# krm01/Snappy.jl

Measured on AMD Instinct MI355X. Metric: GB/s compressed+decompressed (batched blocks) at 1/2/4/8 GPUs; % HBM peak, higher is better.
Workload: dtype u8; 1 GPU; configs 2+3: 10000 x 64 KiB text blocks per GPU, fast-mode compress + uncompress round trip per step; blocks_per_gpu=10000, block_bytes=65536, parallelism=dp1 (blocks sharded per rank, RCCL size all-gather)

## Files before the change

snappy.jl_amd/csrc/sm_compress_sc.hip:

```cpp
#include "sm_device.h"
#include "sm_internal.h"

namespace sm {

constexpr uint32_t kScS = 1024;
constexpr uint32_t kScC = kScS / 64;
constexpr uint32_t kScG = kScS / 64;
constexpr uint32_t kScW = 16;
constexpr uint32_t kScWorkers = kScW - 1;
#ifndef SC_RING
#define SC_RING 16
#endif
constexpr uint32_t kScRing = SC_RING;
static_assert((kScRing & (kScRing - 1)) == 0, "the span kernel's slot sequence needs a power of 2");
constexpr uint32_t kScSlot = 1088;
constexpr uint32_t kScThreads = 64 * kScW;
constexpr uint32_t kScTabBits = 13;
constexpr uint32_t kScTabWords = 1u << kScTabBits;
constexpr uint32_t kScExt = 17;
constexpr uint32_t kScMaxL = 255;
#ifndef SC_SPIN_BITS
#define SC_SPIN_BITS 22
#endif
constexpr uint32_t kScSpinMax = 1u << SC_SPIN_BITS;
static_assert(kScC == 16 && kScG == 16, "a lane's 16 positions: one u16 mask, one 16-byte row");

#ifndef SC_CB
#define SC_CB 2
#endif
#ifndef SC_FAR
#define SC_FAR 256
#endif
constexpr uint32_t kMaskPasses = 16;
#ifndef SC_WPRIO
#define SC_WPRIO 3
#endif
#ifndef SC_TPRIO
#define SC_TPRIO 3
#endif
#ifndef SC_TSLEEP
#define SC_TSLEEP 1
#endif
#ifndef SC_WSLEEP
#define SC_WSLEEP 1
#endif


struct ScWaveLds {
  uint8_t L[kScS];
  uint16_t O[kScS];
};
struct ScLds {
  uint8_t pre[16];
  uint8_t blk[kBlockSize + 64];
  uint32_t T[kScTabWords + 4];
  ScWaveLds w[kScWorkers];
  uint8_t ring[kScRing][kScSlot];
  uint32_t rsize[kScRing];
  uint32_t rseq[kScRing];
  uint32_t ins;
  uint32_t next;
  uint32_t err;
};
static_assert(sizeof(ScLds) <= 160 * 1024, "LDS");
static_assert(sizeof(ScWaveLds) % 32 == 0 && offsetof(ScLds, w) % 32 == 0 && offsetof(ScWaveLds, O) % 32 == 0,
              "rows are 32-byte aligned (section C's O addresses XOR the swizzle into bits 2..4)");
static_assert(kScSlot % 16 == 0 && offsetof(ScLds, ring) % 16 == 0, "slots are 16-byte aligned");
static_assert(kScSlot == kSpanSlot, "the host sizes part pitches by the staging slot");

template <typename Pred>
__device__ __attribute__((always_inline)) inline uint32_t sc_wait(uint32_t* p, Pred pred, uint32_t& err, uint32_t code) {
  uint32_t v;
  for (uint32_t it = 0; !pred(v = uniform(__hip_atomic_load(p, __ATOMIC_ACQUIRE, __HIP_MEMORY_SCOPE_WORKGROUP))); ++it) {
    if (it > kScSpinMax) {
      err |= code;
      break;
    }
    if (SC_WSLEEP) __builtin_amdgcn_s_sleep(SC_WSLEEP);
  }
  return v;
}


__device__ inline uint32_t sc_ld32(const uint8_t* blk, uint32_t a) { return *reinterpret_cast<const uint32_t*>(blk + a); }


__device__ inline uint32_t sc_abyte(uint32_t hi, uint32_t lo, uint32_t s) { return __builtin_amdgcn_alignbyte(hi, lo, s); }

__device__ inline uint32_t sc_ld32u(const uint8_t* blk, uint32_t p) {
  const uint32_t* w = reinterpret_cast<const uint32_t*>(blk + (p & ~3u));
  return sc_abyte(w[1], w[0], p);
}

__device__ inline uint4 sc_ld128(const uint8_t* blk, uint32_t p) {
  const uint32_t* w = reinterpret_cast<const uint32_t*>(blk + (p & ~3u));
  const uint32_t s = p;
  const uint32_t w0 = w[0], w1 = w[1], w2 = w[2], w3 = w[3], w4 = w[4];
  return make_uint4(__builtin_amdgcn_alignbyte(w1, w0, s), __builtin_amdgcn_alignbyte(w2, w1, s),
                    __builtin_amdgcn_alignbyte(w3, w2, s), __builtin_amdgcn_alignbyte(w4, w3, s));
}

__device__ inline uint32_t sc_diff8(uint32_t a0, uint32_t a1, uint32_t b0, uint32_t b1) {
  const uint64_t d = ((uint64_t)(a1 ^ b1) << 32) | (a0 ^ b0);
  return d ? (uint32_t)__builtin_ctzll(d) >> 3 : 8u;
}

__device__ inline uint4 sc_trim(uint4 v, uint32_t len) {
  const uint64_t mlo = len >= 8 ? ~0ull : (1ull << (8 * (len & 7))) - 1;
  const uint64_t mhi = len >= 16 ? ~0ull : (len <= 8 ? 0ull : (1ull << (8 * (len & 7))) - 1);
  return make_uint4(v.x & (uint32_t)mlo, v.y & (uint32_t)(mlo >> 32), v.z & (uint32_t)mhi, v.w & (uint32_t)(mhi >> 32));
}

__device__ inline uint4 sc_trim1(uint4 v, uint32_t len) {
  uint32_t l8 = len << 3;
  asm("" : "+v"(l8));
  uint64_t mlo, mhi;
  asm("v_lshrrev_b64 %0, %1, -1" : "=v"(mlo) : "v"(64 - min(l8, 64u)));
  asm("v_lshrrev_b64 %0, %1, -1" : "=v"(mhi) : "v"(128 - l8));
  const bool hi = len > 8;
  return make_uint4(v.x & (uint32_t)mlo, v.y & (uint32_t)(mlo >> 32), hi ? v.z & (uint32_t)mhi : 0u,
                    hi ? v.w & (uint32_t)(mhi >> 32) : 0u);
}

__device__ inline void sc_lds_or(uint32_t a, uint4 v) {
  const uint32_t wa = (a - 1u) & ~3u, t = 0u - a;
  const uint32_t u0 = __builtin_amdgcn_alignbyte(v.x, 0u, t);
  const uint32_t u1 = __builtin_amdgcn_alignbyte(v.y, v.x, t);
  const uint32_t u2 = __builtin_amdgcn_alignbyte(v.z, v.y, t);
  const uint32_t u3 = __builtin_amdgcn_alignbyte(v.w, v.z, t);
  const uint32_t u4 = __builtin_amdgcn_alignbyte(0u, v.w, t);
  asm volatile("ds_or_b32 %0, %1\nds_or_b32 %0, %2 offset:4\nds_or_b32 %0, %3 offset:8\nds_or_b32 %0, %4 offset:12\n"
               "ds_or_b32 %0, %5 offset:16"
               : : "v"(wa), "v"(u0), "v"(u1), "v"(u2), "v"(u3), "v"(u4) : "memory");
}

__device__ inline void sc_lds_orn(uint32_t a, uint4 v, uint32_t nb) {
  const uint32_t wa = (a - 1u) & ~3u, t = 0u - a, d = a - wa;
  const uint32_t u0 = __builtin_amdgcn_alignbyte(v.x, 0u, t);
  const uint32_t u1 = __builtin_amdgcn_alignbyte(v.y, v.x, t);
  asm volatile("ds_or_b32 %0, %1" : : "v"(wa), "v"(u0) : "memory");
  asm volatile("ds_or_b32 %0, %1 offset:4" : : "v"(wa), "v"(u1) : "memory");
  if (d + nb > 8) {
    const uint32_t u2 = __builtin_amdgcn_alignbyte(v.z, v.y, t);
    const uint32_t u3 = __builtin_amdgcn_alignbyte(v.w, v.z, t);
    const uint32_t u4 = __builtin_amdgcn_alignbyte(0u, v.w, t);
    asm volatile("ds_or_b32 %0, %1 offset:8\nds_or_b32 %0, %2 offset:12\nds_or_b32 %0, %3 offset:16"
                 : : "v"(wa), "v"(u2), "v"(u3), "v"(u4) : "memory");
  }
}

__device__ inline void sc_lds_or3(uint32_t a, uint32_t cv) {
  const uint32_t wa = (a - 1u) & ~3u, t = 0u - a;
  const uint32_t lo = __builtin_amdgcn_alignbyte(cv, 0u, t), hi = __builtin_amdgcn_alignbyte(0u, cv, t);
  asm volatile("ds_or_b32 %0, %1\nds_or_b32 %0, %2 offset:4" : : "v"(wa), "v"(lo), "v"(hi) : "memory");
}

__device__ inline uint4 sc_prepend(uint4 v, uint32_t tag, uint32_t t) {
  if (t == 0) return v;
  const uint32_t s = 4 - t;
  return make_uint4(__builtin_amdgcn_alignbyte(v.x, tag << (8 * s), s), __builtin_amdgcn_alignbyte(v.y, v.x, s),
                    __builtin_amdgcn_alignbyte(v.z, v.y, s), __builtin_amdgcn_alignbyte(v.w, v.z, s));
}

__device__ inline TagBytes sc_run_tag(uint32_t len) {
  __builtin_assume(len >= 1 && len <= kScS);
  return literal_tag(len, kLiteralStd);
}

__device__ inline uint32_t sc_hash_bucket(uint32_t w) {
  uint32_t h;
  asm("v_bfe_u32 %0, %1, %2, %3" : "=v"(h) : "v"(w * kHashMul), "n"(32 - kScTabBits), "n"(kScTabBits));
  return h;
}

__device__ inline uint32_t sc_select(uint64_t m, uint32_t a, uint32_t b) {
  uint32_t r;
  asm("v_cndmask_b32_e64 %0, %1, %2, %3" : "=v"(r) : "v"(b), "v"(a), "s"(m));
  return r;
}

__device__ inline uint32_t sc_sel(uint32_t c, uint32_t a, uint32_t b) { return c ? a : b; }

__device__ inline uint32_t sc_extend(const uint8_t* blk, uint32_t q, uint32_t off, uint32_t L, uint32_t cap) {
  for (;;) {
    const uint4 x = sc_ld128(blk, q + L), y = sc_ld128(blk, q + L - off);
    const uint32_t f0 = sc_diff8(x.x, x.y, y.x, y.y);
    const uint32_t fb = f0 < 8 ? f0 : 8u + sc_diff8(x.z, x.w, y.z, y.w);
    L = min(L + fb, cap);
    if (fb < 16 || L >= cap) return L;
  }
}

__device__ inline uint32_t sc_ffbl(uint32_t x) {
  uint32_t r;
  asm("v_ffbl_b32 %0, %1" : "=v"(r) : "v"(x));
  return r;
}

__device__ __attribute__((always_inline)) inline uint32_t sc_eq16(uint32_t X0, uint32_t X1, uint32_t X2, uint32_t X3,
                                                                  const uint32_t* w, uint32_t s) {
  const uint32_t a0 = w[0], a1 = w[1], a2 = w[2], a3 = w[3], a4 = w[4];
  const uint32_t b0 = sc_ffbl(X0 ^ __builtin_amdgcn_alignbyte(a1, a0, s));
  const uint32_t b1 = sc_ffbl(X1 ^ __builtin_amdgcn_alignbyte(a2, a1, s)) | 32u;
  const uint32_t b2 = sc_ffbl(X2 ^ __builtin_amdgcn_alignbyte(a3, a2, s)) | 64u;
  const uint32_t b3 = sc_ffbl(X3 ^ __builtin_amdgcn_alignbyte(a4, a3, s)) | 96u;
  return min(min(b0, b1), min(min(b2, b3), 128u)) >> 3;
}


__device__ __attribute__((always_inline)) inline uint32_t sc_eq12x(const uint8_t* blk, uint32_t x, uint32_t y) {
  const uint32_t* a = reinterpret_cast<const uint32_t*>(blk + (x & ~3u));
  const uint32_t* b = reinterpret_cast<const uint32_t*>(blk + (y & ~3u));
  const uint32_t a0 = a[0], a1 = a[1], a2 = a[2], a3 = a[3];
  const uint32_t b0 = b[0], b1 = b[1], b2 = b[2], b3 = b[3];
  const uint32_t f0 = sc_ffbl(sc_abyte(a1, a0, x) ^ sc_abyte(b1, b0, y));
  const uint32_t f1 = sc_ffbl(sc_abyte(a2, a1, x) ^ sc_abyte(b2, b1, y)) | 32u;
  const uint32_t f2 = sc_ffbl(sc_abyte(a3, a2, x) ^ sc_abyte(b3, b2, y)) | 64u;
  return min(min(f0, f1), min(f2, 104u)) >> 3;
}

__device__ inline uint32_t scan_max_dpp(uint32_t v) {
  v = max(v, (uint32_t)__builtin_amdgcn_update_dpp(0u, v, 0x111, 0xf, 0xf, true));
  v = max(v, (uint32_t)__builtin_amdgcn_update_dpp(0u, v, 0x112, 0xf, 0xf, true));
  v = max(v, (uint32_t)__builtin_amdgcn_update_dpp(0u, v, 0x114, 0xf, 0xf, true));
  v = max(v, (uint32_t)__builtin_amdgcn_update_dpp(0u, v, 0x118, 0xf, 0xf, true));
  v = max(v, (uint32_t)__builtin_amdgcn_update_dpp(0u, v, 0x142, 0xa, 0xf, false));
  v = max(v, (uint32_t)__builtin_amdgcn_update_dpp(0u, v, 0x143, 0xc, 0xf, false));
  return v;
}

__device__ inline uint32_t sc_bits(uint32_t a, uint32_t b) { return ((1u << b) - 1u) & ~((1u << a) - 1u); }

struct ScToks {
  uint32_t t[4];
  uint32_t n;
};

__device__ __attribute__((always_inline)) inline uint32_t sc_next_block(const CompressArgs& a, uint32_t from, uint32_t g,
                                                                   uint32_t lane) {
  for (uint32_t b0 = from; b0 < a.nblk; b0 += 64 * g) {
    const uint32_t bb = b0 + lane * g;
    const bool todo = bb < a.nblk && (!a.screened || a.out_len[bb] == kScreenTodo);
    const uint64_t m = ballot(todo);
    if (m) return b0 + ctz64(m) * g;
  }
  return a.nblk;
}

template <int kDense>
__device__ __attribute__((always_inline)) inline void sc_superchunk(ScLds& S, const uint32_t k, const uint32_t n,
                                                                   const uint32_t wave, const uint32_t lane_in) {
  uint32_t lane = lane_in;
  asm volatile("" : "+v"(lane));
  ScWaveLds& Wl = S.w[wave];
  const uint32_t sc0 = k * kScS, sce = min(sc0 + kScS, n);
  const uint32_t Tbase = lds_addr(S.T);
  uint32_t ha[kScG], hvv[kScG], wq[kScG];
  const uint32_t ql = sc0 + lane, qa = ql & ~3u, qb = ql;
  const uint32_t hv0 = ql, hv1 = ql << 16;
#pragma unroll
  for (int g = 0; g < (int)kScG; ++g) {
    const uint32_t w = sc_abyte(sc_ld32(S.blk, qa + 64 * g + 4), sc_ld32(S.blk, qa + 64 * g), qb);
    wq[g] = w;
    ha[g] = Tbase + 4 * sc_hash_bucket(w);
    hvv[g] = (g & 1) ? hv1 + ((64u * g) << 16) : hv0 + 64u * g;
  }
  if (sc0 + kScS + 3 > n) {
    asm volatile("");
#pragma unroll
    for (int g = 0; g < (int)kScG; ++g) ha[g] = ql + 64 * g + 4 <= n ? ha[g] : Tbase + 4 * kScTabWords;
  }
  const uint32_t mk0 = 0xffffu, mk1 = 0xffff0000u;
  __builtin_amdgcn_s_setprio(SC_TPRIO);
  for (uint32_t it = 0; uniform(__hip_atomic_load(&S.ins, __ATOMIC_RELAXED, __HIP_MEMORY_SCOPE_WORKGROUP)) != k; ++it) {
    if (it > kScSpinMax) {
      S.err |= 1;
      break;
    }
    if (SC_TSLEEP) __builtin_amdgcn_s_sleep(SC_TSLEEP);
  }
  __builtin_amdgcn_s_setprio(3);
  const uint32_t tok_a = lds_addr(&S.ins), tok_v = k + 1;
  uint32_t r[kScG];
  asm volatile(
      "ds_mskor_rtn_b32 %0, %16, %32, %34\n"
      "ds_mskor_rtn_b32 %1, %17, %33, %35\n"
      "ds_mskor_rtn_b32 %2, %18, %32, %36\n"
      "ds_mskor_rtn_b32 %3, %19, %33, %37\n"
      "ds_mskor_rtn_b32 %4, %20, %32, %38\n"
      "ds_mskor_rtn_b32 %5, %21, %33, %39\n"
      "ds_mskor_rtn_b32 %6, %22, %32, %40\n"
      "ds_mskor_rtn_b32 %7, %23, %33, %41\n"
      "ds_mskor_rtn_b32 %8, %24, %32, %42\n"
      "ds_mskor_rtn_b32 %9, %25, %33, %43\n"
      "ds_mskor_rtn_b32 %10, %26, %32, %44\n"
      "ds_mskor_rtn_b32 %11, %27, %33, %45\n"
      "ds_mskor_rtn_b32 %12, %28, %32, %46\n"
      "ds_mskor_rtn_b32 %13, %29, %33, %47\n"
      "ds_mskor_rtn_b32 %14, %30, %32, %48\n"
      "ds_mskor_rtn_b32 %15, %31, %33, %49\n"
      "ds_write_b32 %50, %51\n"
      "s_waitcnt lgkmcnt(0)"
      : "=&v"(r[0]), "=&v"(r[1]), "=&v"(r[2]), "=&v"(r[3]), "=&v"(r[4]), "=&v"(r[5]), "=&v"(r[6]), "=&v"(r[7]),
        "=&v"(r[8]), "=&v"(r[9]), "=&v"(r[10]), "=&v"(r[11]), "=&v"(r[12]), "=&v"(r[13]), "=&v"(r[14]), "=&v"(r[15])
      : "v"(ha[0]), "v"(ha[1]), "v"(ha[2]), "v"(ha[3]), "v"(ha[4]), "v"(ha[5]), "v"(ha[6]), "v"(ha[7]), "v"(ha[8]),
        "v"(ha[9]), "v"(ha[10]), "v"(ha[11]), "v"(ha[12]), "v"(ha[13]), "v"(ha[14]), "v"(ha[15]), "v"(mk0), "v"(mk1),
        "v"(hvv[0]), "v"(hvv[1]), "v"(hvv[2]), "v"(hvv[3]), "v"(hvv[4]), "v"(hvv[5]), "v"(hvv[6]), "v"(hvv[7]),
        "v"(hvv[8]), "v"(hvv[9]), "v"(hvv[10]), "v"(hvv[11]), "v"(hvv[12]), "v"(hvv[13]), "v"(hvv[14]), "v"(hvv[15]),
        "v"(tok_a), "v"(tok_v)
      : "memory");
  __builtin_amdgcn_s_setprio(0);

  uint64_t mbs[kScG];
  uint8_t* const Ob8 = reinterpret_cast<uint8_t*>(Wl.O);
  const uint32_t Orel = 32 * (lane >> 4) + 2 * (lane & 15);
  if constexpr (kDense) {
#pragma unroll
    for (int g = 0; g < (int)kScG; ++g) {
      const uint32_t q = sc0 + 64 * g + lane;
      const uint32_t sh = 16 * (g & 1);
      const uint32_t ca = (r[g] >> sh) & 0xffffu, cb = (r[g] >> (16 - sh)) & 0xffffu;
      const uint32_t c1 = max(ca, cb), c2 = min(ca, cb);
      const bool ok1 = c1 < q;
      const uint32_t d1 = q - c1, d2 = q - c2;
      uint16_t* const Og = reinterpret_cast<uint16_t*>(Ob8 + (Orel ^ (4u * (g & 7))) + 128u * g);
      const uint32_t r4 = 4 * g + (lane >> 4), i = lane & 15;
      const uint4 X = sc_ld128(S.blk, q);
      uint32_t lw1 = sc_eq16(X.x, X.y, X.z, X.w, reinterpret_cast<const uint32_t*>(S.blk + (c1 & ~3u)), c1);
      uint32_t lw2 = sc_eq16(X.x, X.y, X.z, X.w, reinterpret_cast<const uint32_t*>(S.blk + (c2 & ~3u)), c2);
      asm("" : "+v"(lw1), "+v"(lw2));
      const uint32_t l1 = ok1 ? lw1 : 0u, l2 = ok1 ? lw2 : 0u;
      const bool take2 = l2 == l1 ? (l2 >= 4 && d1 < (uint32_t)SC_FAR) : l2 > l1;
      const uint32_t l = take2 ? l2 : l1;
      const uint32_t avail = sce - q;
      const uint32_t enc = l < 4 ? 0u : ((l == 16 && avail > 16) ? kScExt : min(l, avail));
      *Og = (uint16_t)(take2 ? d2 : d1);
      Wl.L[16 * r4 + 4 * ((i >> 2) ^ ((g >> 1) & 3)) + (i & 3)] = (uint8_t)enc;
      mbs[g] = ballot(l >= 4);
    }
  } else {
#pragma unroll
    for (int g0 = 0; g0 < (int)kScG; g0 += SC_CB) {
      uint32_t c1s[SC_CB], c2s[SC_CB], v1s[SC_CB], v2s[SC_CB];
#pragma unroll
      for (int j = 0; j < SC_CB; ++j) {
        const int g = g0 + j;
        const uint32_t sh = 16 * (g & 1);
        const uint32_t ca = (r[g] >> sh) & 0xffffu, cb = (r[g] >> (16 - sh)) & 0xffffu;
        c1s[j] = max(ca, cb);
        c2s[j] = min(ca, cb);
        v1s[j] = sc_ld32u(S.blk, c1s[j]);
        v2s[j] = sc_ld32u(S.blk, c2s[j]);
      }
#pragma unroll
      for (int j = 0; j < SC_CB; ++j) asm("" : "+v"(v1s[j]), "+v"(v2s[j]));
#pragma unroll
      for (int j = 0; j < SC_CB; ++j) {
        const int g = g0 + j;
        const uint32_t q = sc0 + 64 * g + lane;
        const uint32_t c1 = c1s[j], c2 = c2s[j], w = wq[g];
        const bool ok1 = c1 < q;
        const uint32_t d1 = q - c1, d2 = q - c2;
        uint16_t* const Og = reinterpret_cast<uint16_t*>(Ob8 + (Orel ^ (4u * (g & 7))) + 128u * g);
        const uint64_t OK = ballot(ok1);
        const uint64_t M1 = ballot(v1s[j] == w) & OK, M2 = ballot(v2s[j] == w) & OK;
        const uint64_t U = M2 & (~M1 | ballot(d1 < (uint32_t)SC_FAR));
        *Og = (uint16_t)sc_select(U, d2, d1);
        mbs[g] = M1 | M2;
      }
    }
  }
  uint32_t mdw = 0;
#define SC_WL(g)                                                                                  \
  asm volatile("v_writelane_b32 %0, %1, %2" : "+v"(mdw) : "s"((uint32_t)mbs[g]), "n"(2 * (g)));   \
  asm volatile("v_writelane_b32 %0, %1, %2" : "+v"(mdw) : "s"((uint32_t)(mbs[g] >> 32)), "n"(2 * (g) + 1));
  SC_WL(0) SC_WL(1) SC_WL(2) SC_WL(3) SC_WL(4) SC_WL(5) SC_WL(6) SC_WL(7)
  SC_WL(8) SC_WL(9) SC_WL(10) SC_WL(11) SC_WL(12) SC_WL(13) SC_WL(14) SC_WL(15)
#undef SC_WL
  __atomic_signal_fence(__ATOMIC_SEQ_CST);

  const uint32_t c0 = sc0 + kScC * lane;
  const uint32_t ce = c0 < sce ? min(c0 + kScC, sce) : c0;
  const uint32_t nroom = c0 + 3 < sce ? min(sce - c0 - 3, 16u) : 0u;
  const uint32_t mask16 = (__shfl(mdw, (int)(lane >> 1), 64) >> (16 * (lane & 1))) & ((1u << nroom) - 1u);
  const uint32_t osw2 = ((lane >> 2) & 7) << 1, lsw4 = ((lane >> 3) & 3) << 2;
  const uint16_t* const Orow = Wl.O + 16 * lane;
  auto offAt = [&](uint32_t i) -> uint32_t { return Orow[i ^ osw2]; };
  uint8_t* const Lrow = Wl.L + 16 * lane;
  uint32_t xpos = 16, xlen = 0;
  auto walk = [&](auto kStop, uint32_t sr, uint32_t stop, uint32_t& path, uint32_t& mpos, uint32_t& pend)
      __attribute__((always_inline)) {
    const uint32_t m0 = sr < 16 ? mask16 >> sr : 0u;
    uint32_t i = sr + sc_ffbl(m0);
    path = 0;
    mpos = 16;
    uint32_t last = 16, lastL = 0;
    bool act = m0 != 0;
    while (act) {
      if constexpr (decltype(kStop)::value) {
        if ((stop >> i) & 1u) {
          mpos = i;
          break;
        }
      }
      path |= 1u << i;
      last = i;
      uint32_t enc;
      if constexpr (kDense) {
        enc = Lrow[i ^ lsw4];
      } else {
        const uint32_t q = c0 + i, off = offAt(i);
        const uint32_t p = q - off;
        enc = min(4u + sc_eq12x(S.blk + 4, q, p), sce - q);
        Lrow[i ^ lsw4] = (uint8_t)enc;
      }
      lastL = enc;
      const uint32_t t = i + min(enc, 16u);
      const uint32_t m = mask16 >> t;
      i = t + sc_ffbl(m);
      act = m != 0;
    }
    pend = ce;
    if (last < 16) {
      uint32_t L = lastL;
      const bool ext = L == kScExt;
      if (last + min(L, 16u) >= 16) {
        if (ballot(ext)) {
          if (ext) {
            if (xpos != last) {
              xlen = sc_extend(S.blk, c0 + last, offAt(last), 16u, min(kScMaxL, sce - (c0 + last)));
              xpos = last;
            }
            L = xlen;
          }
        }
        pend = c0 + last + L;
      }
    }
  };
  const bool row = c0 < sce;
  uint32_t s = c0, e, P;
  {
    uint32_t mp;
    walk(std::false_type{}, row ? 0u : 16u, 0u, P, mp, e);
    if (!row) e = c0;
  }
  for (uint32_t pass = 0;; ++pass) {
    const uint32_t pe = __builtin_amdgcn_update_dpp(0u, scan_max_dpp(e), 0x138, 0xf, 0xf, false);
    const uint32_t st = lane == 0 ? sc0 : pe;
    uint32_t sn = st;
    bool chg = st != s;
    if (!ballot(chg)) break;
    if (pass < kMaskPasses) {
      uint64_t cov = ballot(st >= ce);
      for (int it = 0; cov && it < 3; ++it) {
        const uint32_t x = sn >= ce ? 0u : e;
        const uint32_t pm = __builtin_amdgcn_update_dpp(0u, scan_max_dpp(x), 0x138, 0xf, 0xf, false);
        sn = lane == 0 ? sc0 : pm;
        const uint64_t c = ballot(sn >= ce);
        if (c == cov) break;
        cov = c;
      }
      chg = sn != s;
      if (!ballot(chg)) {
        sn = st;
        chg = st != s;
      }
    }

    const bool inrow = chg && sn < ce;
    uint32_t nP, mp, ne;
    walk(std::true_type{}, inrow ? sn - c0 : 16u, P, nP, mp, ne);
    if (chg) {
      s = sn;
      if (!inrow) {
        P = 0;
        e = sn;
      } else if (mp == 16) {
        P = nP;
        e = ne;
      } else {
        P = nP | (P & ~sc_bits(0, mp));
      }
    }
  }
  auto getL = [&](uint32_t i) -> uint32_t { return Lrow[i ^ lsw4]; };
  ScToks tk;
  {
    uint32_t pm = P;
    tk.n = (uint32_t)__builtin_popcount(P);
#pragma unroll
    for (int j = 0; j < 4; ++j) {
      const uint32_t i = pm ? (uint32_t)__builtin_ctz(pm) : 0u;
      pm &= pm - 1;
      uint32_t L = getL(i);
      L = L == kScExt ? xlen : L;
      const uint32_t off = offAt(i);
      tk.t[j] = off | (L << 16) | (i << 24);
    }
  }

  const bool live = s >= c0 && s < ce;
  uint32_t lead = 0, body = 0, trail = 0;
  {
    uint32_t p = s;
#pragma unroll
    for (int j = 0; j < 4; ++j) {
      const bool has = (uint32_t)j < tk.n;
      const uint32_t tv = tk.t[j];
      const uint32_t q = c0 + (tv >> 24), L = (tv >> 16) & 0xffu, run = q - p;
      if (j == 0)
        lead = sc_sel(has, run, 0u);
      else
        body += sc_sel(has && run, run + 1, 0u);
      body += sc_sel(has, copy_tag_bytes(tv & 0xffffu, L), 0u);
      p = sc_sel(has, q + L, p);
    }
    trail = (live && p < ce) ? ce - p : 0u;
    lead = tk.n == 0 ? trail : lead;
  }
  const uint32_t ptrail = __builtin_amdgcn_update_dpp(0u, trail, 0x138, 0xf, 0xf, false);
  const bool cont = ptrail > 0 && lead > 0;
  const bool mid = cont && tk.n == 0;
  const uint32_t Cs = scan_dpp(cont ? lead : 0u);
  const uint64_t above = ballot(!mid) & (~1ull << lane);
  const uint32_t fn = above ? ctz64(above) : 63u;
  const uint32_t Cf = __shfl(Cs, fn, 64);
  const bool starts = trail > 0 && !mid;
  const uint32_t merged = starts ? trail + Cf - Cs : 0u;
  const uint32_t mts = sc_run_tag(merged ? merged : 1u).size;
  uint32_t size;
  if (tk.n == 0)
    size = lead == 0 ? 0u : (cont ? lead : mts + trail);
  else
    size = (lead ? (cont ? lead : 1u + lead) : 0u) + body + (trail ? mts + trail : 0u);
  const uint32_t incl = scan_dpp(size);
  const uint32_t total = readlane(incl, 63);

  const uint32_t slot = k % kScRing;
  (void)sc_wait(&S.rseq[slot], [&](uint32_t v) { return v == k; }, S.err, 2u);

  uint8_t* const stg = S.ring[slot];
  {
    for (uint32_t u = lane; 16 * u < total; u += 64) reinterpret_cast<uint4*>(stg)[u] = make_uint4(0, 0, 0, 0);
    const uint32_t stga = lds_addr(stg);
    uint32_t at = incl - size, p = s;
#pragma unroll
    for (int j = 0; j < 4; ++j) {
      if ((uint32_t)j < tk.n) {
        const uint32_t tv = tk.t[j];
        const uint32_t q = c0 + (tv >> 24), L = (tv >> 16) & 0xffu, off = tv & 0xffffu;
        const uint32_t run = q - p;
        const uint32_t ts = (j == 0 && cont) ? 0u : 1u;
        const uint32_t len = run ? ts + run : 0u;
        if (ballot(len != 0)) {
          uint4 v = sc_ld128(S.blk - 4, p + 3);
          v.x = ts ? ((v.x & ~0xffu) | literal_tag1(run)) : v.x;
          if (run) sc_lds_orn(stga + at + ts - 1u, sc_trim1(v, run + 1), run + 1);
        }
        at += len;
        if (L <= 64) {
          const TagBytes c = copy_piece(off, L);
          sc_lds_or3(stga + at, (uint32_t)c.bytes);
          at += c.size;
        } else {
          uint32_t R = L;
          do {
            const uint32_t l = copy_piece_len(R);
            const TagBytes c = copy_piece(off, l);
            sc_lds_or3(stga + at, (uint32_t)c.bytes);
            at += c.size;
            R -= l;
          } while (R);
        }
        p = q + L;
      }
    }
    if (live && p < ce) {
      const uint32_t run = ce - p;
      uint32_t tag = 0, ts = 0;
      if (!(tk.n == 0 && cont)) {
        const TagBytes lt = sc_run_tag(merged);
        tag = (uint32_t)lt.bytes;
        ts = lt.size;
      }
      sc_lds_orn(stga + at, sc_trim(sc_prepend(sc_ld128(S.blk, p), tag, ts), min(ts + run, 16u)), min(ts + run, 16u));
      if (ts + run > 16) sc_lds_or(stga + at + 16, sc_trim(sc_ld128(S.blk, p + 16 - ts), ts + run - 16));
    }
  }
  __hip_atomic_store(&S.rsize[slot], total + 1, __ATOMIC_RELEASE, __HIP_MEMORY_SCOPE_WORKGROUP);
}

typedef uint32_t __attribute__((ext_vector_type(4), aligned(1))) sc_u128u;
__device__ __attribute__((always_inline)) inline void sc_copy_out(uint8_t* const g, const uint8_t* stg, uint32_t len,
                                                                 uint32_t lane) {
  const uint32_t nu = len >> 4;
  for (uint32_t u = lane; u < nu; u += 64) {
    const uint4 v = reinterpret_cast<const uint4*>(stg)[u];
    sc_u128u x;
    x.x = v.x, x.y = v.y, x.z = v.z, x.w = v.w;
    *reinterpret_cast<sc_u128u*>(g + 16 * u) = x;
  }
  if (lane < (len & 15u)) g[16 * nu + lane] = stg[16 * nu + lane];
}

__device__ __attribute__((always_inline)) inline void sc_writer(ScLds& S, uint32_t n, uint8_t* const dst, uint32_t hv,
                                                               uint32_t k0, uint32_t k1, bool whole,
                                                               uint32_t* len_out, uint32_t lane) {
  uint32_t o = hv, err = 0;
  uint32_t vpre = 0;
  for (uint32_t k = k0; k < k1; ++k) {
    const uint32_t slot = k % kScRing;
    const uint32_t sz =
        (vpre ? vpre : sc_wait(&S.rsize[slot], [](uint32_t v) { return v != 0; }, err, 4u)) - 1;
    if (err) break;
    vpre = k + 1 < k1 ? uniform(__hip_atomic_load(&S.rsize[(k + 1) % kScRing], __ATOMIC_ACQUIRE,
                                                    __HIP_MEMORY_SCOPE_WORKGROUP))
                        : 0u;
    sc_copy_out(dst + o, S.ring[slot], sz, lane);
    o += sz;
    __hip_atomic_store(&S.rsize[slot], 0u, __ATOMIC_RELAXED, __HIP_MEMORY_SCOPE_WORKGROUP);
    __hip_atomic_store(&S.rseq[slot], k + kScRing, __ATOMIC_RELEASE, __HIP_MEMORY_SCOPE_WORKGROUP);
  }
  const uint32_t len = block_literal_bytes(n, false);
  if (whole && !err && n && o > hv + len) {
    uint8_t* const g = dst + hv;
    const uint32_t tb = len - n;
    const uint32_t ad = (uint32_t)((uintptr_t)g & 15);
    uint4* const g16 = reinterpret_cast<uint4*>(g - ad);
    const uint32_t u1 = (len + ad) >> 4;
    const uint32_t ua = (tb + ad + 15) >> 4;
    for (uint32_t u = ua + lane; u < u1; u += 64) g16[u] = sc_ld128(S.blk, 16 * u - ad - tb);
    const uint32_t he = ua < u1 ? 16 * ua - ad : len;
    const uint32_t te = ua < u1 ? 16 * u1 - ad : len;
    for (uint32_t j = lane; j < he + (len - te); j += 64) {
      const uint32_t jj = j < he ? j : te + (j - he);
      g[jj] = jj < tb ? block_literal_head_byte(n, false, jj) : S.blk[jj - tb];
    }
    o = hv + len;
  }
  err |= uniform(__hip_atomic_load(&S.err, __ATOMIC_RELAXED, __HIP_MEMORY_SCOPE_WORKGROUP));
  if (lane == 0) *len_out = err ? kOutLenError | err : o;
}

__device__ __attribute__((always_inline)) inline void sc_stage_block(ScLds& S, const uint8_t* src, uint32_t n, bool there,
                                                                    uint8_t* dst, uint32_t hv) {
  const uint32_t tid = threadIdx.x;
  if (there) {
  } else if (((uintptr_t)src & 15) == 0) {
    const uint4* s16 = reinterpret_cast<const uint4*>(src);
    uint4* d16 = reinterpret_cast<uint4*>(S.blk);
    const uint32_t n16 = n >> 4;
    for (uint32_t k = tid; k < n16; k += kScThreads) d16[k] = s16[k];
    for (uint32_t k = (n & ~15u) + tid; k < n; k += kScThreads) S.blk[k] = src[k];
  } else {
    for (uint32_t k = tid; k < n; k += kScThreads) S.blk[k] = src[k];
  }
  if (tid < 64) S.blk[n + tid] = 0;
  uint4* t16 = reinterpret_cast<uint4*>(S.T);
  for (uint32_t k = tid; k < 4 * kScTabWords / 16; k += kScThreads) t16[k] = make_uint4(0, 0, 0, 0);
  if (tid < hv) dst[tid] = varint_byte(n, tid, hv);
}

__device__ __attribute__((always_inline)) inline void sc_reset_handoff(ScLds& S, uint32_t k0) {
  const uint32_t lane = threadIdx.x & 63;
  if (uniform(threadIdx.x >> 6) != 0) return;
  if (lane < kScRing) {
    S.rsize[lane] = 0;
    S.rseq[lane] = k0 + ((lane - k0) & (kScRing - 1));
  }
  if (lane == 0) {
    S.ins = k0;
    S.next = 64 * k0;
    S.err = 0;
  }
}

template <int kDense>
__device__ __attribute__((always_inline)) inline void sc_span_item(ScLds& S, const CompressArgs& a, const ScSpan& sp,
                                                                  const uint32_t item) {
  const uint32_t tid = threadIdx.x;
  const uint32_t wave = uniform(tid >> 6);
  const uint32_t lane = tid & 63;
  const uint32_t b = item / sp.parts, j = item % sp.parts;
  if (b >= a.nblk) return;
  uint32_t* const plen = sp.part_len + item;
  const uint32_t n = a.in_len[b];
  if (n > kBlockSize) {
    if (tid == 0) *plen = j == 0 ? kNotABlock : 0u;
    return;
  }
  const uint32_t nsc = (n + kScS - 1) / kScS;
  const uint32_t k0 = j * sp.span, k1 = min(k0 + sp.span, nsc);
  const bool todo = !a.screened || a.out_len[b] == kScreenTodo;
  if (!todo || k0 >= k1) {
    if (tid == 0) *plen = (!todo && j == 0) ? (sp.blk_pitch ? kPartScreened : a.out_len[b]) : 0u;
    return;
  }
  const uint8_t* const src = a.in + a.in_off[b];
  uint8_t* const dst = a.out + (sp.blk_pitch ? b * sp.blk_pitch : a.out_off[b]) + (uint64_t)j * sp.pitch;
  const uint32_t hv = (a.header && j == 0) ? varint_len(n) : 0u;
  sc_stage_block(S, src, n, false, dst, hv);
  sc_reset_handoff(S, k0);
  __syncthreads();
  const uint32_t pe = kScS * k0;
  const uint32_t sub = lane & 15, gq = lane >> 4;
  for (int ph = 1; ph >= 0; --ph) {
    for (uint32_t i = wave; 128 * (4 * i) < pe; i += kScW) {
      const uint32_t G = 2 * (4 * i + gq) + (uint32_t)ph;
      const uint32_t q = 64 * G + 4 * sub;
      if (q >= pe) continue;
      const uint32_t d0 = sc_ld32(S.blk, q), d1 = sc_ld32(S.blk, q + 4);
      uint32_t* t[4];
#pragma unroll
      for (uint32_t j = 0; j < 4; ++j) {
        const uint32_t w = j ? __builtin_amdgcn_alignbyte(d1, d0, j) : d0;
        t[j] = &S.T[(w * kHashMul) >> (32 - kScTabBits)];
      }
      if (ph) {
#pragma unroll
        for (uint32_t j = 0; j < 4; ++j)
          if (q + j + 4 <= n) __hip_atomic_fetch_max(t[j], (q + j) << 16, __ATOMIC_RELAXED, __HIP_MEMORY_SCOPE_WORKGROUP);
      } else {
        uint32_t hi[4];
#pragma unroll
        for (uint32_t j = 0; j < 4; ++j) hi[j] = __hip_atomic_load(t[j], __ATOMIC_RELAXED, __HIP_MEMORY_SCOPE_WORKGROUP);
#pragma unroll
        for (uint32_t j = 0; j < 4; ++j)
          if (q + j + 4 <= n)
            __hip_atomic_fetch_max(t[j], (hi[j] & 0xffff0000u) | (q + j), __ATOMIC_RELAXED, __HIP_MEMORY_SCOPE_WORKGROUP);
      }
    }
    __syncthreads();
  }
  if (wave == kScWorkers) {
    __builtin_amdgcn_s_setprio(SC_WPRIO);
    sc_writer(S, n, dst, hv, k0, k1, false, plen, lane);
    __builtin_amdgcn_s_setprio(0);
  } else {
    for (;;) {
      const uint32_t k = uniform(__hip_atomic_fetch_add(&S.next, 1u, __ATOMIC_RELAXED, __HIP_MEMORY_SCOPE_WORKGROUP)) >> 6;
      if (k >= k1) break;
      sc_superchunk<kDense>(S, k, n, wave, lane);
    }
  }
}

template <int kDense>
__global__ __launch_bounds__(kScThreads) void k_compress_sc_span(CompressArgs a, ScSpan sp) {
  __shared__ __attribute__((aligned(16))) ScLds S;
  sc_span_item<kDense>(S, a, sp, blockIdx.x);
}

template <int kDense>
__global__ __launch_bounds__(kScThreads) void k_compress_sc(CompressArgs a, uint32_t g, CompressArgs r, ScSpan sp) {
  __shared__ __attribute__((aligned(16))) ScLds S;
  if (blockIdx.x >= g) {
    sc_span_item<kDense>(S, r, sp, blockIdx.x - g);
    return;
  }
  const uint32_t tid = threadIdx.x;
  const uint32_t wave = uniform(tid >> 6);
  const uint32_t lane = tid & 63;
  static_assert(kBlockSize / 16 / kScThreads == 4, "four 16-byte pieces per thread of a full block");
  uint4 pf0, pf1, pf2, pf3;
  uint32_t b = sc_next_block(a, blockIdx.x, g, lane);
  uint32_t n = 0;
  const uint8_t* src = nullptr;
  bool inpf = false;
#define SC_FETCH(bb)                                                              \
  {                                                                               \
    n = (bb) < a.nblk ? a.in_len[bb] : 0u;                                        \
    src = (bb) < a.nblk ? a.in + a.in_off[bb] : nullptr;                          \
    inpf = (bb) < a.nblk && n == kBlockSize && ((uintptr_t)src & 15) == 0;        \
    if (inpf) {                                                                   \
      const uint4* s16 = reinterpret_cast<const uint4*>(src);                     \
      pf0 = s16[tid];                                                             \
      pf1 = s16[tid + kScThreads];                                                \
      pf2 = s16[tid + 2 * kScThreads];                                            \
      pf3 = s16[tid + 3 * kScThreads];                                            \
    }                                                                             \
  }
  SC_FETCH(b)
  while (b < a.nblk) {
    uint8_t* const dst = a.out + a.out_off[b];
    if (n > kBlockSize) {
      if (tid == 0) a.out_len[b] = kNotABlock;
      b = sc_next_block(a, b + g, g, lane);
      SC_FETCH(b)
      continue;
    }
    if (inpf) {
      uint4* d16 = reinterpret_cast<uint4*>(S.blk);
      d16[tid] = pf0;
      d16[tid + kScThreads] = pf1;
      d16[tid + 2 * kScThreads] = pf2;
      d16[tid + 3 * kScThreads] = pf3;
    }
    const uint32_t hv = a.header ? varint_len(n) : 0u;
    sc_stage_block(S, src, n, inpf, dst, hv);
    sc_reset_handoff(S, 0);
    const uint32_t bn = sc_next_block(a, b + g, g, lane);
    __syncthreads();

    const uint32_t nsc = (n + kScS - 1) / kScS;
    if (wave == kScWorkers) {
      __builtin_amdgcn_s_setprio(SC_WPRIO);
      sc_writer(S, n, dst, hv, 0, nsc, true, &a.out_len[b], lane);
      __builtin_amdgcn_s_setprio(0);
    } else {
      for (;;) {
        const uint32_t k = uniform(__hip_atomic_fetch_add(&S.next, 1u, __ATOMIC_RELAXED, __HIP_MEMORY_SCOPE_WORKGROUP)) >> 6;
        if (k >= nsc) break;
        sc_superchunk<kDense>(S, k, n, wave, lane);
      }
    }
    SC_FETCH(bn)
    __syncthreads();
    b = bn;
  }
#undef SC_FETCH
}

hipError_t launch_compress_sc_span(const CompressArgs& a, int mode, const ScSpan& sp, hipStream_t s) {
  if (sp.parts == 0 || sp.span == 0 || sp.parts * sp.span < (kBlockSize + kScS - 1) / kScS ||
      sp.pitch < (uint64_t)sp.span * kScSlot)
    return hipErrorInvalidValue;
  const uint32_t grid = a.nblk * sp.parts;
  if (grid == 0) return hipSuccess;
  if (mode == 2)
    hipLaunchKernelGGL(k_compress_sc_span<1>, dim3(grid), dim3(kScThreads), 0, s, a, sp);
  else
    hipLaunchKernelGGL(k_compress_sc_span<0>, dim3(grid), dim3(kScThreads), 0, s, a, sp);
  return hipGetLastError();
}


hipError_t launch_compress_sc_parts(const CompressArgs& a, const CompressArgs& r, const ScSpan& sp, int mode,
                                    hipStream_t s) {
  const uint32_t g = min(a.nblk, compress_grid());
  const uint32_t items = sp.parts ? r.nblk * sp.parts : 0u;
  if (items && (sp.span == 0 || sp.parts * sp.span < (kBlockSize + kScS - 1) / kScS ||
                sp.pitch < (uint64_t)sp.span * kScSlot || sp.blk_pitch < sp.parts * sp.pitch))
    return hipErrorInvalidValue;
  if (g + items == 0) return hipSuccess;
  if (mode == 2)
    hipLaunchKernelGGL(k_compress_sc<1>, dim3(g + items), dim3(kScThreads), 0, s, a, g, r, sp);
  else
    hipLaunchKernelGGL(k_compress_sc<0>, dim3(g + items), dim3(kScThreads), 0, s, a, g, r, sp);
  return hipGetLastError();
}

hipError_t launch_compress_sc(const CompressArgs& a, int mode, hipStream_t s) {
  return launch_compress_sc_parts(a, CompressArgs{}, ScSpan{}, mode, s);
}

}
```

Measured before the change: 403.4 GB/s.

## Load next block's shares on demand and prefetch descriptors through the writer wave

The whole-block prefetch, where every thread loaded four 16-byte pieces of the next block after the superchunk loop, is replaced by dynamic share claiming. At the start of each block, worker waves atomically grab up to two 4 KiB shares and load them into registers, then store them to LDS. The writer wave now loads candidate descriptors for the block after next (lengths, offsets, screen marks) before it writes. After writing, it picks the next todo block with a ballot and publishes it via LDS, so descriptor lookup no longer sits on the critical path. The load is no longer overlapped with compute in the prior iteration, which may expose fetch latency, and the extra register slots add pressure.

```diff
diff --git a/snappy.jl_amd/csrc/sm_compress_sc.hip b/snappy.jl_amd/csrc/sm_compress_sc.hip
--- a/snappy.jl_amd/csrc/sm_compress_sc.hip
+++ b/snappy.jl_amd/csrc/sm_compress_sc.hip
@@ -38,6 +38,9 @@
 #ifndef SC_TPRIO
 #define SC_TPRIO 3
 #endif
+#ifndef SC_MAX_SHARES
+#define SC_MAX_SHARES 2
+#endif
 #ifndef SC_TSLEEP
 #define SC_TSLEEP 1
 #endif
@@ -61,6 +64,8 @@
   uint32_t ins;
   uint32_t next;
   uint32_t err;
+  uint32_t share;
+  uint32_t nx[6];
 };
 static_assert(sizeof(ScLds) <= 160 * 1024, "LDS");
 static_assert(sizeof(ScWaveLds) % 32 == 0 && offsetof(ScLds, w) % 32 == 0 && offsetof(ScWaveLds, O) % 32 == 0,
@@ -663,7 +668,8 @@
 }
 
 __device__ __attribute__((always_inline)) inline void sc_reset_handoff(ScLds& S, uint32_t k0) {
-  const uint32_t lane = threadIdx.x & 63;
+  uint32_t lane = threadIdx.x & 63;
+  asm volatile("" : "+v"(lane));
   if (uniform(threadIdx.x >> 6) != 0) return;
   if (lane < kScRing) {
     S.rsize[lane] = 0;
@@ -673,6 +679,7 @@
     S.ins = k0;
     S.next = 64 * k0;
     S.err = 0;
+    S.share = 0;
   }
 }
 
@@ -752,6 +759,78 @@
   sc_span_item<kDense>(S, a, sp, blockIdx.x);
 }
 
+struct ScBlk {
+  uint32_t b, n;
+  uint64_t ioff, ooff;
+};
+struct ScCand {
+  uint32_t mark, n;
+  uint64_t ioff, ooff;
+};
+
+__device__ inline uint64_t uniform64(uint64_t v) { return uniform((uint32_t)v) | (uint64_t)uniform((uint32_t)(v >> 32)) << 32; }
+__device__ inline uint64_t readlane64(uint64_t v, uint32_t l) {
+  return readlane((uint32_t)v, l) | (uint64_t)readlane((uint32_t)(v >> 32), l) << 32;
+}
+
+__device__ __attribute__((always_inline)) inline ScBlk sc_blk_scan(const CompressArgs& a, uint32_t from, uint32_t g,
+                                                                  uint32_t lane) {
+  ScBlk r{sc_next_block(a, from, g, lane), 0u, 0u, 0u};
+  if (r.b < a.nblk) {
+    r.n = uniform(a.in_len[r.b]);
+    r.ioff = uniform64(a.in_off[r.b]);
+    r.ooff = uniform64(a.out_off[r.b]);
+  }
+  return r;
+}
+
+constexpr uint32_t kCandDesc = 4;
+__device__ __attribute__((always_inline)) inline ScCand sc_cand_load(const CompressArgs& a, uint32_t from, uint32_t g,
+                                                                    uint32_t lane) {
+  const uint32_t bb = min(from + lane * g, a.nblk - 1);
+  const uint32_t bd = min(from + (lane & (kCandDesc - 1)) * g, a.nblk - 1);
+  return ScCand{a.out_len[bb], a.in_len[bd], a.in_off[bd], a.out_off[bd]};
+}
+
+__device__ __attribute__((always_inline)) inline ScBlk sc_cand_pick(const CompressArgs& a, const ScCand& c, uint32_t from,
+                                                                   uint32_t g, uint32_t lane) {
+  if (from >= a.nblk) return ScBlk{a.nblk, 0u, 0u, 0u};
+  const bool todo = from + lane * g < a.nblk && (!a.screened || c.mark == kScreenTodo);
+  const uint64_t m = ballot(todo);
+  if (m == 0) return sc_blk_scan(a, from + 64 * g, g, lane);
+  const uint32_t l = ctz64(m);
+  if (l >= kCandDesc) return sc_blk_scan(a, from + l * g, g, lane);
+  return ScBlk{from + l * g, readlane(c.n, l), readlane64(c.ioff, l), readlane64(c.ooff, l)};
+}
+
+__device__ inline void sc_put_nx(ScLds& S, const ScBlk& k) {
+  S.nx[0] = k.b;
+  S.nx[1] = k.n;
+  S.nx[2] = (uint32_t)k.ioff;
+  S.nx[3] = (uint32_t)(k.ioff >> 32);
+  S.nx[4] = (uint32_t)k.ooff;
+  S.nx[5] = (uint32_t)(k.ooff >> 32);
+}
+__device__ inline ScBlk sc_get_nx(const ScLds& S) {
+  return ScBlk{uniform(S.nx[0]), uniform(S.nx[1]), uniform(S.nx[2]) | (uint64_t)uniform(S.nx[3]) << 32,
+               uniform(S.nx[4]) | (uint64_t)uniform(S.nx[5]) << 32};
+}
+
+__device__ inline bool sc_blk_shares(const CompressArgs& a, const ScBlk& k) {
+  return k.b < a.nblk && k.n == kBlockSize && ((uintptr_t)(a.in + k.ioff) & 15) == 0;
+}
+
+constexpr uint32_t kMaxShares = SC_MAX_SHARES;
+constexpr uint32_t kShareSlots = kMaxShares ? kMaxShares : 1;
+constexpr uint32_t kShares = kScW;
+constexpr uint32_t kShareU = kBlockSize / 16 / kShares;
+static_assert(kShareU == 4 * 64, "four 16-byte pieces per lane of a share");
+typedef uint32_t __attribute__((ext_vector_type(4))) sc_u128;
+struct ScShare {
+  sc_u128 p0, p1, p2, p3;
+  uint32_t s;
+};
+
 template <int kDense>
 __global__ __launch_bounds__(kScThreads) void k_compress_sc(CompressArgs a, uint32_t g, CompressArgs r, ScSpan sp) {
   __shared__ __attribute__((aligned(16))) ScLds S;
@@ -759,55 +838,94 @@
     sc_span_item<kDense>(S, r, sp, blockIdx.x - g);
     return;
   }
-  const uint32_t tid = threadIdx.x;
-  const uint32_t wave = uniform(tid >> 6);
-  const uint32_t lane = tid & 63;
-  static_assert(kBlockSize / 16 / kScThreads == 4, "four 16-byte pieces per thread of a full block");
-  uint4 pf0, pf1, pf2, pf3;
-  uint32_t b = sc_next_block(a, blockIdx.x, g, lane);
-  uint32_t n = 0;
-  const uint8_t* src = nullptr;
-  bool inpf = false;
-#define SC_FETCH(bb)                                                              \
-  {                                                                               \
-    n = (bb) < a.nblk ? a.in_len[bb] : 0u;                                        \
-    src = (bb) < a.nblk ? a.in + a.in_off[bb] : nullptr;                          \
-    inpf = (bb) < a.nblk && n == kBlockSize && ((uintptr_t)src & 15) == 0;        \
-    if (inpf) {                                                                   \
-      const uint4* s16 = reinterpret_cast<const uint4*>(src);                     \
-      pf0 = s16[tid];                                                             \
-      pf1 = s16[tid + kScThreads];                                                \
-      pf2 = s16[tid + 2 * kScThreads];                                            \
-      pf3 = s16[tid + 3 * kScThreads];                                            \
-    }                                                                             \
-  }
-  SC_FETCH(b)
-  while (b < a.nblk) {
-    uint8_t* const dst = a.out + a.out_off[b];
-    if (n > kBlockSize) {
-      if (tid == 0) a.out_len[b] = kNotABlock;
-      b = sc_next_block(a, b + g, g, lane);
-      SC_FETCH(b)
-      continue;
-    }
+  const uint32_t wave = uniform(threadIdx.x >> 6);
+  uint32_t lane = threadIdx.x & 63;
+  static_assert(kMaxShares <= 8, "slots sh0..7");
+  static_assert(kMaxShares == 0 || kMaxShares * kScWorkers >= kShares, "the workers can hold a block");
+#define SC_SLOTS(X) X(0, sh0) X(1, sh1) X(2, sh2) X(3, sh3) X(4, sh4) X(5, sh5) X(6, sh6) X(7, sh7)
+#define SC_FETCH_SHARE(i, sh, s_)                                                                        \
+  {                                                                                                      \
+    const sc_u128* s16 = reinterpret_cast<const sc_u128*>(a.in + cur.ioff) + kShareU * (s_) + lane;      \
+    sh.s = (s_);                                                                                         \
+    sh.p0 = s16[0];                                                                                      \
+    sh.p1 = s16[64];                                                                                     \
+    sh.p2 = s16[128];                                                                                    \
+    sh.p3 = s16[192];                                                                                    \
+    ns = (i) + 1;                                                                                        \
+  }
+#define SC_SKIP_OVERSIZE(blk, one)                                   \
+  while ((blk).b < a.nblk && (blk).n > kBlockSize) {                 \
+    if (one) a.out_len[(blk).b] = kNotABlock;                        \
+    (blk) = sc_blk_scan(a, (blk).b + g, g, lane);                    \
+  }
+  ScBlk cur = sc_blk_scan(a, blockIdx.x, g, lane);
+  SC_SKIP_OVERSIZE(cur, threadIdx.x == 0)
+  {
+    ScBlk nxt = sc_blk_scan(a, cur.b + g, g, lane);
+    SC_SKIP_OVERSIZE(nxt, threadIdx.x == 0)
+    if (threadIdx.x == 0) {
+      S.share = 0;
+      sc_put_nx(S, nxt);
+    }
+  }
+  __syncthreads();
+  while (cur.b < a.nblk) {
+    asm volatile("" : "+v"(lane));
+    const uint32_t tid = 64 * wave + lane;
+    ScShare sh0, sh1, sh2, sh3, sh4, sh5, sh6, sh7;
+#define SC_NEW_SHARE(i, sh)                              \
+  sh.p0 = __builtin_nondeterministic_value(sh.p0);       \
+  sh.p1 = __builtin_nondeterministic_value(sh.p1);       \
+  sh.p2 = __builtin_nondeterministic_value(sh.p2);       \
+  sh.p3 = __builtin_nondeterministic_value(sh.p3);       \
+  sh.s = 0;
+    SC_SLOTS(SC_NEW_SHARE)
+#undef SC_NEW_SHARE
+    uint32_t ns = 0;
+    const bool inpf = sc_blk_shares(a, cur);
+    if (kMaxShares == 0) {
+      if (inpf) SC_FETCH_SHARE(0, sh0, wave)
+    } else if (inpf && wave != kScWorkers) {
+#define SC_TAKE_SHARE(i, sh)                                                                                               \
+  if (i < kMaxShares && ns == i) {                                 \
+    const uint32_t s = uniform(__hip_atomic_fetch_add(&S.share, 1u, __ATOMIC_RELAXED, __HIP_MEMORY_SCOPE_WORKGROUP)) >> 6; \
+    if (s < kShares) SC_FETCH_SHARE(i, sh, s)                                                                              \
+  }
+      SC_SLOTS(SC_TAKE_SHARE)
+#undef SC_TAKE_SHARE
+    }
+    __syncthreads();
+
+    const uint32_t n = cur.n;
+    uint8_t* const dst = a.out + cur.ooff;
     if (inpf) {
-      uint4* d16 = reinterpret_cast<uint4*>(S.blk);
-      d16[tid] = pf0;
-      d16[tid + kScThreads] = pf1;
-      d16[tid + 2 * kScThreads] = pf2;
-      d16[tid + 3 * kScThreads] = pf3;
+      sc_u128* const d16 = reinterpret_cast<sc_u128*>(S.blk) + lane;
+#define SC_PUT_SHARE(i, sh)                     \
+  if (i < kShareSlots && i < ns) {              \
+    sc_u128* const d = d16 + kShareU * sh.s;    \
+    d[0] = sh.p0;                               \
+    d[64] = sh.p1;                              \
+    d[128] = sh.p2;                             \
+    d[192] = sh.p3;                             \
+  }
+      SC_SLOTS(SC_PUT_SHARE)
+#undef SC_PUT_SHARE
     }
     const uint32_t hv = a.header ? varint_len(n) : 0u;
-    sc_stage_block(S, src, n, inpf, dst, hv);
+    sc_stage_block(S, a.in + cur.ioff, n, inpf, dst, hv);
     sc_reset_handoff(S, 0);
-    const uint32_t bn = sc_next_block(a, b + g, g, lane);
+    const ScBlk nxt = sc_get_nx(S);
     __syncthreads();
 
     const uint32_t nsc = (n + kScS - 1) / kScS;
     if (wave == kScWorkers) {
       __builtin_amdgcn_s_setprio(SC_WPRIO);
-      sc_writer(S, n, dst, hv, 0, nsc, true, &a.out_len[b], lane);
+      const ScCand cand = sc_cand_load(a, nxt.b + g, g, lane);
+      sc_writer(S, n, dst, hv, 0, nsc, true, &a.out_len[cur.b], lane);
       __builtin_amdgcn_s_setprio(0);
+      ScBlk after = nxt.b < a.nblk ? sc_cand_pick(a, cand, nxt.b + g, g, lane) : nxt;
+      SC_SKIP_OVERSIZE(after, lane == 0)
+      if (lane == 0) sc_put_nx(S, after);
     } else {
       for (;;) {
         const uint32_t k = uniform(__hip_atomic_fetch_add(&S.next, 1u, __ATOMIC_RELAXED, __HIP_MEMORY_SCOPE_WORKGROUP)) >> 6;
@@ -815,11 +933,11 @@
         sc_superchunk<kDense>(S, k, n, wave, lane);
       }
     }
-    SC_FETCH(bn)
-    __syncthreads();
-    b = bn;
-  }
-#undef SC_FETCH
+    cur = nxt;
+  }
+#undef SC_SKIP_OVERSIZE
+#undef SC_FETCH_SHARE
+#undef SC_SLOTS
 }
 
 hipError_t launch_compress_sc_span(const CompressArgs& a, int mode, const ScSpan& sp, hipStream_t s) {
```

Result: no change. 404.6 GB/s (median of 6 runs) (+0.3%).
